# Dostenlinus/Aiyagari-HARK

Hardware: AMD Instinct MI355X
Metric: GE solves/sec (Table II sweep); agent-periods/sec; % HBM roofline (higher is better)
Workload: dtype f64

## Files before the change

### aiyagari_hark_amd/csrc/ge_resident.hip

```cpp
#include "common.h"
#include "egm_common.h"
#include "ge_search.h"
#include "hist_bicg.h"
#include "hist_cluster.h"
#include "internal.h"

#include <algorithm>
#include <cmath>

namespace aiy {

constexpr int kGeTHMax = 1024;
constexpr int kGeWavesMax = kGeTHMax / kWave;
constexpr int kGeMaxTiles = 16;
constexpr int kGeBufs = 5;
constexpr int kGeAaM = 3;
constexpr int kGeAaHist = kGeAaM + 2;
#ifdef AIY_DIAG_NO_FUSEA
constexpr bool kGeFuseA = false;
#else
constexpr bool kGeFuseA = true;
#endif
#ifndef AIY_FUSEA_KC2
#define AIY_FUSEA_KC2 0
#endif
constexpr bool kGeFuseAKc2 = AIY_FUSEA_KC2 != 0;
template <int NW>
constexpr size_t ge_egm_lds() { return (size_t)NW * (8 * kTile + 4 * kWin) * sizeof(double); }

struct GeCalDev {
  double alpha, delta, disc, r_lo, r_hi;
};

struct GeState;
struct GeRun {
  int n_cal, S, n_a, G, nj, cap, n_work;
  const double* a_grid;
  const double* P;
  const double* lab;
  const double* beta;
  const double* crra;
  const GeCalDev* cal;
  int method;
  double r_tol, egm_tol, hist_tol;
  int max_steps, max_cyc, max_hist;
  int warm_hist, warm_egm, secant, loose, extrap;
  int extrap_period;
  int aa_period;
  double* aah;
  int logsec;
  double loose_hist;
  double* qb;
  int* ainv;
  double* tab;
  double* mass;
  double* pmass;
  double* pg;
  int* lo;
  double* wlo;
  double* slab;
  int* span;
  unsigned* ctr;
  unsigned long long* gran;
  const int* cal_ids;
  GeState* saved;
  const int* resume;
  unsigned* done_ctr;
  int stop_at;
  int* out_done;
  unsigned* err;
  double* out_r;
  double* out_K;
  double* out_Ks;
  int* out_steps;
  int* out_cyc;
  int* out_its;
  int* out_status;
  double* out_prof;
  double* out_evlog;
};
constexpr int kGeProf = 8;
constexpr int kGeEvLog = 32;
constexpr int kGeEvRec = 6;

struct GeState {
  GeEval ev;
  GeEvalOpts opt;
  double Ks, dist, lam_prev, fext;
  int status, n, stop, nan_stop, moved, extrap;
  int in_hist;
  int buf[kGeBufs];
  long long cyc_sum, its_sum;
  unsigned long long t_egm, t_lot, t_hist, t_k, t0, t_ev0;
  unsigned nc_prev[2];
  unsigned nbc;
};

template <int TH>
__device__ __forceinline__ bool ge_reduce(unsigned long long* gran, int G, int w, unsigned& ne, const double* vals,
                                          int nv, unsigned kmax, double (*s_part)[kGeWavesMax], double* s_res,
                                          int* s_flag, unsigned* err) {
  asm volatile("s_waitcnt vmcnt(0)" ::: "memory");
  return hc_reduce<TH>(gran, G, w, ne, vals, nv, kmax, s_part, s_res, s_flag, err, [] {});
}

template <int SMAX, int NW, typename Sink, typename Begin, typename End>
__device__ __forceinline__ void ge_rows_pass(int S, int n_a, int j0, int j1, const double* __restrict__ a_grid,
                                             const double* __restrict__ src_m, const double* __restrict__ src_c,
                                             double R, const double* s_Wl, int* s_hint, double* lds_win,
                                             Sink&& sink, Begin&& begin, End&& end) {
  const int tid = threadIdx.x, lane = tid & (kWave - 1);
  const int wv = __builtin_amdgcn_readfirstlane(tid / kWave);
  const int n = n_a, n1 = n_a + 1;
  const int ntile = (j1 - j0 + kTile - 1) / kTile;
  double* X = lds_win + (size_t)wv * 4 * kWin;
  double* Y = X + kWin;
  double* XB = X + 2 * kWin;
  double* YB = X + 3 * kWin;
#pragma unroll 1
  for (int tile = wv; tile < ntile; tile += NW) {
    const int jr = j0 + tile * kTile + lane;
    const int j = jr < j1 ? jr : j1 - 1;
    const double a = a_grid[j];
    int* hint = s_hint + tile * SMAX;
    auto fetch = [&](int r, RowWin& wn) {
      const int rr = r < S ? r : S - 1;
      load_win<true>(src_m + (size_t)rr * n1, src_c + (size_t)rr * n1, n, win_base(hint[rr], n1), lane, wn);
    };
    unsigned redo = 0u;
    auto step_unit = [&](int u, const RowWin& wa, const RowWin& wb) {
      const int ra = 2 * u, rb = 2 * u + 1;
      if (ra >= S) return;
      const bool has_b = rb < S;
      const int rbb = has_b ? rb : ra;
      const bool na = __any(stage_win(wa, n, X, Y, lane));
      const bool nb = __any(stage_win(wb, n, XB, YB, lane));
      __builtin_amdgcn_fence(__ATOMIC_RELEASE, "wavefront");
      __builtin_amdgcn_wave_barrier();
      __builtin_amdgcn_fence(__ATOMIC_ACQUIRE, "wavefront");
      const double qa = R * a + s_Wl[ra];
      const double qb = R * a + s_Wl[rbb];
      int lba, lbb;
      bool oka, okb;
      const double fa = search_win(wa.base, na, n, qa, X, Y, lba, oka);
      const double fb = search_win(wb.base, nb, n, qb, XB, YB, lbb, okb);
      hint[ra] = __builtin_amdgcn_readfirstlane(lba);
      if (has_b) hint[rb] = __builtin_amdgcn_readfirstlane(lbb);
      if (__any(!oka)) redo |= 1u << ra;
      else sink(tile, jr, j, ra, qa, fa);
      if (has_b) {
        if (__any(!okb)) redo |= 1u << rb;
        else sink(tile, jr, j, rb, qb, fb);
      }
    };
    RowWin a0, b0, a1, b1;
    fetch(0, a0);
    fetch(1, b0);
    begin(tile, j);
#pragma unroll 1
    for (int u = 0; 2 * u < S; u += 2) {
      fetch(2 * u + 2, a1);
      fetch(2 * u + 3, b1);
      step_unit(u, a0, b0);
      fetch(2 * u + 4, a0);
      fetch(2 * u + 5, b0);
      step_unit(u + 1, a1, b1);
    }
#pragma unroll 1
    while (redo != 0u) {
      const int s = __builtin_ctz(redo);
      redo &= redo - 1u;
      const double q = R * a + s_Wl[s];
      int lb;
      const double f = interp_row_global_agent(src_m + (size_t)s * n1, src_c + (size_t)s * n1, n, q, lb);
      hint[s] = __builtin_amdgcn_readfirstlane(lb);
      sink(tile, jr, j, s, q, f);
    }
    end(tile, j, a);
  }
// ... 450 lines not shown
  pf[1] = st.t_lot * 0.01;
  pf[2] = st.t_hist * 0.01;
  pf[3] = st.t_k * 0.01;
  pf[4] = (__builtin_amdgcn_s_memrealtime() - st.t0) * 0.01;
  pf[5] = (double)st.cyc_sum;
  pf[6] = (double)st.its_sum;
  pf[7] = (double)st.ev.steps;
}

template <int SMAX, int SC, int KC, int TH, bool PULL>
__global__ __launch_bounds__(TH) void ge_cluster_kernel(GeRun g) {
  constexpr int NW = TH / kWave;
  static_assert(SMAX <= kGeSmax, "file-scope LDS sized for kGeSmax states");
  GeState& st = ge_st;

  const int per = gridDim.x >> 3;
  const int u = (blockIdx.x & 7) * per + (blockIdx.x >> 3);
  if (u >= g.n_work) return;
  const int G = g.G, S = g.S, n_a = g.n_a;
  const int tid = threadIdx.x;
  GeCtx cx;
  cx.G = G; cx.S = S; cx.n_a = n_a;
  cx.lc = u / G; cx.w = u - cx.lc * G;
  const int lc = cx.lc, w = cx.w, cal = g.cal_ids[lc];
  cx.cal = cal;
  cx.j0 = w * g.nj; cx.j1 = min(cx.j0 + g.nj, n_a);
  const int j0 = cx.j0, j1 = cx.j1;
  cx.a_grid = g.a_grid + (size_t)cal * n_a;
  cx.beta = g.beta[cal]; cx.gam = g.crra[cal];
  const GeCalDev cd = g.cal[cal];
  cx.tab_sz = (size_t)S * (n_a + 1);
  cx.tab = g.tab + (size_t)cal * kGeBufs * 2 * cx.tab_sz;
  const size_t row0 = (size_t)cal * S * n_a;
  cx.X = g.mass + row0;
  cx.PX = g.pmass + row0;
  cx.LO = g.lo + row0;
  cx.WL = g.wlo + row0;
  cx.ctr = g.ctr + (size_t)lc * kHcCtrStride;
  cx.cw = reinterpret_cast<unsigned long long*>(cx.ctr + 2);
  cx.gran = g.gran + (size_t)lc * 2 * G * kHcRedRec;
  cx.aah = g.aah + (size_t)cal * kGeAaHist * S * n_a;
  cx.err = g.err;
  unsigned nb = 0, ne = 0;
  const int pk = cx.gam == 1.0 ? 1 : (cx.gam == 3.0 ? 3 : (cx.gam == 5.0 ? 5 : 0));

  for (int q = tid; q < S * S; q += TH) ge_s_Pe[q] = g.P[(size_t)cal * S * S + q];
  for (int q = tid; q < kGeMaxTiles * SMAX; q += TH) ge_s_hint[q] = -1;
  if (tid == 0) {
    if (g.resume[cal]) {
      st = g.saved[cal];
      st.t0 = __builtin_amdgcn_s_memrealtime() - st.t0;
    } else {
      st.ev.init(ge_eval_opts(g), cd.r_lo, cd.r_hi);
      st.Ks = 0.0;
      st.in_hist = 0;
      st.status = 0;
      st.cyc_sum = st.its_sum = 0;
      for (int b = 0; b < kGeBufs; ++b) st.buf[b] = b;
      st.t_egm = st.t_lot = st.t_hist = st.t_k = 0ull;
      st.t0 = __builtin_amdgcn_s_memrealtime();
    }
    st.opt = ge_eval_opts(g);
    st.nc_prev[0] = st.nc_prev[1] = 0u;
    st.nbc = 0u;
  }
  __syncthreads();

  bool stopped = false;
  while ((!st.ev.rs.done && st.ev.steps < g.max_steps) || st.ev.final_ks) {
    if (g.stop_at > 0 && st.ev.steps > 0 && !st.in_hist) {
      unsigned flag = 0u, dlt = 0u;
      if (tid == 0)
        flag = __hip_atomic_load(to_global(g.done_ctr), __ATOMIC_RELAXED, __HIP_MEMORY_SCOPE_AGENT) >=
                       (unsigned)g.stop_at ? 1u : 0u;
      if (!ge_vote(cx, g.err, flag, dlt)) return;
      if (tid == 0) st.stop = dlt != 0u;
      __syncthreads();
      if (st.stop) {
        stopped = true;
        break;
      }
    }
    unsigned long long tp = __builtin_amdgcn_s_memrealtime();
    if (tid == 0 && !st.in_hist) st.t_ev0 = tp;
    if (!st.in_hist) {
      if (tid == 0) {
        st.ev.plan(st.opt, cd.alpha, cd.delta);
        st.extrap = g.extrap;
        st.moved = 0;
      }
      __syncthreads();
      if (tid < S) ge_s_Wl[tid] = st.ev.wage * g.lab[(size_t)cal * S + tid];
      const double R = st.ev.R, theta = st.ev.theta;
      const bool secant = st.ev.secant != 0, warm = st.ev.warm_egm != 0;
      const int b_cur = st.buf[2], b_prev = st.buf[3], b_init = st.buf[4];
      if (secant) ge_secant_tables<TH>(cx, b_cur, b_prev, b_init, theta);
      tp = __builtin_amdgcn_s_memrealtime();
      GeHhArgs ha;
      ha.tab = to_global(cx.tab); ha.aah = to_global(cx.aah); ha.ctr = to_global(cx.ctr); ha.err = to_global(g.err);
      ha.gran = to_global(cx.gran); ha.a_grid = to_global(cx.a_grid);
      ha.init_m = to_global((const double*)(secant ? cx.tabm(b_init) : (warm ? cx.tabm(b_cur) : nullptr)));
      ha.init_c = to_global((const double*)(secant ? cx.tabc(b_init) : (warm ? cx.tabc(b_cur) : nullptr)));
      ha.beta = cx.beta; ha.gam = cx.gam; ha.R = R;
      ha.j0 = j0; ha.j1 = j1; ha.w = w; ha.G = G; ha.S = S; ha.n_a = n_a;
      ha.opt = {g.max_cyc, g.aa_period, g.extrap_period};
      ha.dyn_lds = hk_lds_addr(ge_dyn);
      const int final_buf = pk == 1   ? ge_household_isolated<SMAX, SC, 1, TH>(ha, &nb, &ne)
                            : pk == 3 ? ge_household_isolated<SMAX, SC, 3, TH>(ha, &nb, &ne)
                            : pk == 5 ? ge_household_isolated<SMAX, SC, 5, TH>(ha, &nb, &ne)
                                      : ge_household_isolated<SMAX, SC, 0, TH>(ha, &nb, &ne);
      if (final_buf < 0) return;
      if (tid == 0) {
        const unsigned long long tn = __builtin_amdgcn_s_memrealtime();
        st.t_egm += tn - tp;
        st.cyc_sum += st.n;
        const int fb = final_buf;
        const int other = st.buf[0] == fb ? st.buf[1] : st.buf[0];
        const int old_prev = st.buf[3];
        st.buf[3] = st.buf[2];
        st.buf[2] = fb;
        st.buf[0] = other;
        st.buf[1] = old_prev;
      }
      __syncthreads();
      tp = __builtin_amdgcn_s_memrealtime();
      ge_lottery_fn<SMAX, NW>(S, n_a, j0, j1, cx.a_grid, cx.tabm(st.buf[2]), cx.tabc(st.buf[2]), R, st.ev.steps > 0,
                              cx.LO, cx.WL, PULL);
      ge_mass_start<TH>(cx, st.ev.fresh_mass != 0, warm, secant, theta);
      __syncthreads();
      if (tid == 0) {
        const unsigned long long tn = __builtin_amdgcn_s_memrealtime();
        st.t_lot += tn - tp;
        tp = tn;
      }
    }
    int mv;
    {
      HkArgs hk;
      hk.G = G; hk.S = S; hk.n_a = n_a; hk.cap = g.cap; hk.w = w; hk.j0 = j0; hk.j1 = j1;
      hk.LO = to_global((const int*)cx.LO); hk.WL = to_global((const double*)cx.WL); hk.X = to_global(cx.X);
      hk.Pg = to_global(g.pg + row0); hk.Vg = to_global((double*)nullptr);
      hk.slab_cl = to_global(g.slab + (size_t)lc * G * 2 * g.cap);
      hk.span_cl = to_global(g.span + (size_t)lc * G * SMAX * 4);
      hk.ctr = to_global(cx.ctr); hk.gran = to_global(cx.gran); hk.Pc = to_global(g.P + (size_t)cal * S * S);
      hk.max_iter = g.max_hist; hk.err = to_global(g.err);
      hk.tol = st.ev.htol;
      hk.stop_ctr = to_global((const unsigned*)(g.stop_at > 0 ? g.done_ctr : nullptr));
      hk.stop_at = (unsigned)g.stop_at;
      hk.Qg = to_global(g.qb + row0);
      hk.Ainv = to_global(g.ainv + (size_t)cal * S * (n_a + 1));
      hk.lottery_fresh = true;
      hk.dyn_lds = hk_lds_addr(ge_dyn);
      if constexpr (PULL) mv = hk_solve_inlined<SMAX, KC, TH, true, false, SC>(hk, &nb, &ne);
      else mv = hk_solve_isolated<SMAX, KC, TH, false, (KC == 1 || kGeFuseAKc2) && kGeFuseA, SC>(hk, &nb, &ne);
    }
    if (mv == -1) return;
    if (tid == 0) {
      const unsigned long long tn = __builtin_amdgcn_s_memrealtime();
      st.t_hist += tn - tp;
      tp = tn;
    }
    if (mv <= -2) {
      if (tid == 0) {
        st.its_sum += -mv - 2;
        st.in_hist = 1;
        if (w == 0) __hip_atomic_fetch_add(to_global(g.done_ctr + 1), 1u, __ATOMIC_RELAXED, __HIP_MEMORY_SCOPE_AGENT);
      }
      __syncthreads();
      stopped = true;
      break;
    }
    if (tid == 0) st.in_hist = 0;
    if (!ge_capital<TH>(cx, ne, g.err)) return;
    const bool fin = st.ev.final_ks != 0;
    if (tid == 0) {
      const double Ks = ge_s_res[0];
      if (w == 0 && st.ev.steps < kGeEvLog && !fin) {
        double* ev = g.out_evlog + ((size_t)cal * kGeEvLog + st.ev.steps) * kGeEvRec;
        ev[0] = st.ev.rs.x;
        ev[1] = (Ks - st.ev.Kd) / st.ev.Kd;
        ev[2] = (double)st.n;
        ev[3] = (double)mv;
        ev[4] = (double)st.ev.loose;
        ev[5] = (double)(__builtin_amdgcn_s_memrealtime() - st.t_ev0) * 0.01;
      }
      st.its_sum += mv;
      if (mv >= g.max_hist) st.status |= 2;
    }
    if (fin) {
      if (tid == 0) st.Ks = ge_s_res[0];
      __syncthreads();
      break;
    }
    if (tid == 0) {
      st.ev.accept(ge_s_res[0]);
      st.Ks = ge_s_res[0];
      st.t_k += __builtin_amdgcn_s_memrealtime() - tp;
    }
    __syncthreads();
  }
  if (stopped) {
    if (w == 0 && tid == 0) {
      st.t0 = __builtin_amdgcn_s_memrealtime() - st.t0;
      g.saved[cal] = st;
      g.out_done[cal] = 0;
    }
    return;
  }
  if (w == 0 && tid == 0) ge_write_out(cx, g, cd);
}

struct GePlan {
  int G = 0, nj = 0, kc = 0, smax = 0, sc = 0, cap = 0, blocks = 0, th = 0;
  size_t lds = 0;
  const void* fn = nullptr;
};

template <int SMAX, int SC, int KC, int TH>
static const void* ge_fn(bool pull) {
  return pull ? reinterpret_cast<const void*>(ge_cluster_kernel<SMAX, SC, KC, TH, true>)
              : reinterpret_cast<const void*>(ge_cluster_kernel<SMAX, SC, KC, TH, false>);
}

static bool ge_make_plan(aiy_handle* h, int n_cal, int S, int n_a, GePlan& p) {
  if (S < 1 || S > kGeSmax || n_a < 2 || n_cal < 1) return false;
  int cus = 0;
  if (hipDeviceGetAttribute(&cus, hipDeviceAttributeMultiprocessorCount, h->device) != hipSuccess || cus < 1) return false;
  if (h->cu_limit > 0) cus = std::min(cus, h->cu_limit);
  const int g_min = (n_a + 2 * 512 - 1) / (2 * 512);
  if (g_min > kHcMaxG || g_min > cus) return false;
  const int g_cap = h->hist_cluster_cap > 0 ? h->hist_cluster_cap : 32;
  int G = std::max(g_min, std::min(std::min(g_cap, kHcMaxG), cus / n_cal));
  G = std::min(G, n_a);
  p.nj = (n_a + G - 1) / G;
  p.G = (n_a + p.nj - 1) / p.nj;
  if (p.G > kHcMaxG) return false;
  if (p.nj > kGeMaxTiles * kTile) return false;
  if ((long long)p.G * n_cal > cus) return false;
  p.th = 512;
  const int th = p.th;
  p.kc = p.nj <= th ? 1 : 2;
  p.smax = S == 7 ? 7 : 8;
  p.sc = S == 7 ? 7 : 0;
  const bool pull = h->hist_pull != 0;
  if (p.sc == 7) p.fn = p.kc == 1 ? ge_fn<7, 7, 1, 512>(pull) : ge_fn<7, 7, 2, 512>(pull);
  else p.fn = p.kc == 1 ? ge_fn<8, 0, 1, 512>(pull) : ge_fn<8, 0, 2, 512>(pull);
  hipFuncAttributes fa;
  if (hipFuncGetAttributes(&fa, p.fn) != hipSuccess) return false;
  int lds_dev = 0;
  if (hipDeviceGetAttribute(&lds_dev, hipDeviceAttributeMaxSharedMemoryPerMultiprocessor, h->device) != hipSuccess)
    return false;
  const size_t lds_total = std::min<size_t>(kHcLdsTotal, (size_t)lds_dev);
  const size_t stat = fa.sharedSizeBytes;
  if (stat + 4096 >= lds_total) return false;
  p.lds = (lds_total - stat - 1024) / 256 * 256;
  const size_t vbytes = (size_t)p.kc * p.smax * th * sizeof(double);
  const size_t egm_lds = ge_egm_lds<8>();
  if (p.lds < egm_lds || p.lds <= vbytes + 4096) return false;
  p.cap = (int)((p.lds - vbytes) / sizeof(double));
  p.blocks = (p.G * n_cal + 7) / 8 * 8;
  return true;
}

struct GeScratch {
  size_t tab, mass, pmass, pg, qb, ainv, lo, wlo, slab, span, ctr, gran, ids, saved, resume, done, err, cal, outd, outi, prof,
      evlog, aah, bytes;
};
static GeScratch ge_scratch_layout(int n_cal, int S, int n_a, int cus, int cap_max) {
  GeScratch L;
  size_t o = 0;
  auto take = [&](size_t bytes) { const size_t at = o; o += (bytes + 255) / 256 * 256; return at; };
  const size_t pts = (size_t)n_cal * S * n_a;
  L.tab = take((size_t)n_cal * kGeBufs * 2 * S * (n_a + 1) * sizeof(double));
  L.mass = take(pts * 8); L.pmass = take(pts * 8); L.pg = take(pts * 8); L.qb = take(pts * 8);
  L.ainv = take((size_t)n_cal * S * (n_a + 1) * sizeof(int));
  L.lo = take(pts * 4); L.wlo = take(pts * 8);
  L.slab = take((size_t)cus * 2 * cap_max * sizeof(double));
  L.span = take((size_t)cus * 8 * 4 * sizeof(int));
  L.ctr = take((size_t)n_cal * kHcCtrStride * sizeof(unsigned));
  L.gran = take((size_t)cus * 2 * kHcRedRec * sizeof(unsigned long long));
  L.ids = take((size_t)n_cal * sizeof(int));
  L.saved = take((size_t)n_cal * sizeof(GeState));
  L.resume = take((size_t)n_cal * sizeof(int));
  L.done = take((size_t)n_cal * sizeof(int));
  L.err = take(256);
  L.cal = take((size_t)n_cal * sizeof(GeCalDev));
  L.outd = take((size_t)n_cal * 3 * sizeof(double));
  L.outi = take((size_t)n_cal * 4 * sizeof(int));
  L.prof = take((size_t)n_cal * kGeProf * sizeof(double));
  L.evlog = take((size_t)n_cal * kGeEvLog * kGeEvRec * sizeof(double));
  L.aah = take((size_t)n_cal * kGeAaHist * S * n_a * sizeof(double));
  L.bytes = o;
  return L;
}

int32_t ge_stationary_resident(aiy_handle* h, const aiy_stationary_model* M, const aiy_ge_options* o, double* r_out,
                               double* K_out, double* Ks_out, int32_t* steps_out, int32_t* cyc_out,
                               int32_t* its_out, int32_t* status_out, hipStream_t st) {
  if (!h->ge_resident || o->accel >= 0) return 0;
  const int n_cal = M->n_cal, S = M->S, n_a = M->n_a;
  GePlan p0;
  if (!ge_make_plan(h, n_cal, S, n_a, p0)) return 0;
  int cus = 0;
  if (hipDeviceGetAttribute(&cus, hipDeviceAttributeMultiprocessorCount, h->device) != hipSuccess) return 0;
  if (h->cu_limit > 0) cus = std::min(cus, h->cu_limit);
  const int cap_max = (int)(kHcLdsTotal / sizeof(double));
  const GeScratch L = ge_scratch_layout(n_cal, S, n_a, cus, cap_max);
// ... 208 lines not shown
```

### aiyagari_hark_amd/csrc/hist_bicg.h

```cpp
#pragma once

#include "common.h"
#include "hist_cluster.h"

namespace aiy {

constexpr int kHkStall = 256;
constexpr double kHkStopSentinel = 1e300;
constexpr int kHkHeavy = 31;
#ifndef AIY_HK_WAVE_CN
#define AIY_HK_WAVE_CN 6
#endif
constexpr int kHkWaveCn = AIY_HK_WAVE_CN;
static_assert(kHcCand <= 32, "covering-span index and count packed in 5 + 6 bits");
__device__ __forceinline__ unsigned short hk_cinfo(int cf, int cn, int hi) {
  return (unsigned short)(cf | (cn << 5) | (hi << 11));
}
__device__ __forceinline__ int hk_cf(int ci) { return ci & 31; }
__device__ __forceinline__ int hk_cn(int ci) { return (ci >> 5) & 63; }
__device__ __forceinline__ int hk_hi(int ci) { return ci >> 11; }

__device__ __forceinline__ double hk_uni(double x) {
  const unsigned long long u = (unsigned long long)__double_as_longlong(x);
  const unsigned lo = (unsigned)__builtin_amdgcn_readfirstlane((int)(unsigned)u);
// ... 544 lines not shown
            const int n1c = a2[u] - a1[u], n0c = a1[u] - a0[u];
            const bool heavy = valid && (n1c + n0c) > kWave;
            double acc = 0.0;
            if (valid && !heavy) {
              if (n1c > 0) acc += wv[u][0] * qv[u][0];
              if (n1c > 1) acc += wv[u][1] * qv[u][1];
              for (int j = a1[u] + 2; j < a2[u]; ++j) acc += w_at(sr, j) * q_at(sr, j);
              if (n0c > 0) acc += (1.0 - wv[u][2]) * qv[u][2];
              if (n0c > 1) acc += (1.0 - wv[u][3]) * qv[u][3];
              for (int j = a0[u] + 2; j < a1[u]; ++j) acc += (1.0 - w_at(sr, j)) * q_at(sr, j);
            }
            unsigned long long hm = __ballot(heavy);
            while (hm) {
              const int h = __builtin_ctzll(hm);
              hm &= hm - 1ull;
              const int b0 = __builtin_amdgcn_readlane(a0[u], h), b1 = __builtin_amdgcn_readlane(a1[u], h),
                        b2 = __builtin_amdgcn_readlane(a2[u], h);
              double pa = 0.0, pb = 0.0;
              for (int j = b1 + lane; j < b2; j += kWave) pa += w_at(sr, j) * q_at(sr, j);
              for (int j = b0 + lane; j < b1; j += kWave) pb += (1.0 - w_at(sr, j)) * q_at(sr, j);
              const double ta = wave_sum_lane63(pa), tb = wave_sum_lane63(pb);
              const double tot = __shfl(ta, kWave - 1, kWave) + __shfl(tb, kWave - 1, kWave);
              if (lane == h) acc = tot;
            }
            T[sr] = acc;
          }
        }
      }
#pragma unroll
      for (int sp = 0; sp < SMAX; ++sp) {
        double pc[SMAX];
        asm volatile("" ::: "memory");
#pragma unroll
        for (int s = 0; s < SMAX; ++s) pc[s] = s_P[s * SMAX + sp];
        double acc = 0.0;
#pragma unroll
        for (int s = 0; s < SMAX; ++s) acc += pc[s] * T[s];
        out[k][sp] = acc;
      }
    }
  };
  auto matvec = [&](const double (&q)[KC][SMAX], double (&out)[KC][SMAX]) -> bool {
    if constexpr (PULL) {
      HK_PH(5);
      stage_q(q);
      HK_PH(1);
      if (!barrier()) return false;
      HK_PH(2);
      pull_mix(out);
      HK_PH(3);
      return true;
    }
    HK_PH(5);
    push(q);
    HK_PH(0);
    const int par = (int)((nb + 1) & 1);
    publish(par);
    HK_PH(1);
    if (!barrier()) return false;
    HK_PH(2);
    gather_mix(par, out);
    HK_PH(3);
    return true;
  };
  auto reduce = [&](double (&vals)[kHcRed], int nv, unsigned kmax, auto&& prefetch) -> bool {
    HK_PH(5);
    hc_wave_parts(vals, nv, kmax, s_part);
    __syncthreads();
    ++ne;
    const unsigned long long tag = hc_red_tag(ne);
    unsigned long long* slot = hc_red_slot(gran, G, ne);
    hc_store_granules<TH>(slot, w, tag, nv, kmax, s_part);
    prefetch();
    if (wid == 0) hc_sweep(slot, G, tag, nv, kmax, s_res, &s_flag, err);
    __syncthreads();
    HK_PH(4);
    return s_flag != 0;
  };
  auto matvec_rp = [&](auto&& do_push, double (&out)[KC][SMAX], const double* vals, int nv, unsigned kmax) -> bool {
    HK_PH(5);
    hc_wave_parts(vals, nv, kmax, s_part);
    do_push();
    HK_PH(0);
    ++ne;
    const unsigned long long tag = hc_red_tag(ne);
    unsigned long long* slot = hc_red_slot(gran, G, ne);
    hc_store_granules<TH>(slot, w, tag, nv, kmax, s_part);
    const int par = (int)((nb + 1) & 1);
    publish(par);
    HK_PH(1);
    if (!barrier()) return false;
    HK_PH(2);
    if (wid == TH / kWave - 1) hc_sweep(slot, G, tag, nv, kmax, s_res, L.s_rok, err);
    gather_mix(par, out);
    __syncthreads();
    HK_PH(3);
    return *L.s_rok != 0;
  };
  auto matvec_r = [&](const double (&q)[KC][SMAX], double (&out)[KC][SMAX], const double* vals, int nv,
                      unsigned kmax) -> bool { return matvec_rp([&] { push(q); }, out, vals, nv, kmax); };
  double rv[KC][SMAX], pv[KC][SMAX], tv[KC][SMAX];
  double* Vl = kVlds ? Tacc + cap : (double*)r.Vg;
  double* Pg = (double*)r.Pg;
  auto vidx = [&](int k, int s) { return (k * SMAX + s) * TH + tid; };
  double part[kHcRed];
  const double tol = r.tol;
  int mv = 0;
  bool restart = true, first = true;
  double rho = 0.0, total0 = 0.0;
  auto own = [&](int jc, int k, int s) { return s < S && jc + k * TH < j1; };
  auto col_act = [&](int jc, bool (&act)[KC]) {
#pragma unroll
    for (int k = 0; k < KC; ++k) act[k] = jc + k * TH < j1;
  };
  bool act[KC];
  unsigned seed = 0;
  auto rh_at = [&](int jc, int k, int s) { return hk_rhat((unsigned)(s * n_a + jc + k * TH) + seed * 0x5BD1E995u); };
  double best = __builtin_inf();
  int mv_best = 0;
  auto gidx = [&](int jc, int k, int s) { return (size_t)s * n_a + jc + k * TH; };
  double* Ug = (double*)r.Qg;
  double pu = 0.0;
  auto make_u = [&]() {
    if constexpr (FUSEA) {
      const int jc = col();
      double acc = 0.0;
#pragma unroll
      for (int k = 0; k < KC; ++k)
#pragma unroll
        for (int s = 0; s < SMAX; ++s) {
          if (own(jc, k, s)) {
            int d;
            double wl;
            if constexpr (kLoReg) {
              d = dreg[k][s];
              wl = wreg[k][s];
            } else {
              d = LO[gidx(jc, k, s)];
              wl = WL[gidx(jc, k, s)];
            }
            double tr = 0.0;
            for (int sp = 0; sp < S; ++sp) {
              const unsigned q = (unsigned)(sp * n_a + d) + seed * 0x5BD1E995u;
              tr += s_P[s * SMAX + sp] * (wl * hk_rhat(q) + (1.0 - wl) * hk_rhat(q + 1u));
            }
            const double u = rh_at(jc, k, s) - tr;
            Ug[gidx(jc, k, s)] = u;
            acc += u * pv[k][s];
          }
        }
      pu = acc;
    }
  };
#ifndef AIY_FUSEA_KC2
#define AIY_FUSEA_KC2 0
#endif
  constexpr bool kUqPre = KC == 1 || AIY_FUSEA_KC2 == 1;
  HK_PH(-1);
  while (true) {
    if (restart) {
      int jc = col();
#pragma unroll
      for (int k = 0; k < KC; ++k)
#pragma unroll
        for (int s = 0; s < SMAX; ++s) {
          const double xv = X[min(s, S - 1) * n_a + min(jc + k * TH, n_a - 1)];
          pv[k][s] = own(jc, k, s) ? xv : 0.0;
        }
      if (!matvec(pv, tv)) return -1;
      ++mv;
      jc = col();
      double rr = 0.0, rm = 0.0, xs = 0.0;
#pragma unroll
      for (int k = 0; k < KC; ++k)
#pragma unroll
        for (int s = 0; s < SMAX; ++s) {
          rv[k][s] = tv[k][s] - pv[k][s];
          if (own(jc, k, s)) {
            rr += rh_at(jc, k, s) * rv[k][s];
            rm = nan_max(rm, fabs(rv[k][s]));
            xs += pv[k][s];
          }
        }
      part[0] = rr;
      part[1] = rm;
      part[2] = xs;
      if (!reduce(part, 3, 2u, [] {})) return -1;
      rho = s_res[0];
      if (mv == 1) total0 = s_res[2];
      if (s_res[1] < tol || mv >= r.max_iter) {
        const double scale = total0 / s_res[2];
#pragma unroll
        for (int k = 0; k < KC; ++k)
#pragma unroll
          for (int s = 0; s < SMAX; ++s)
            if (own(jc, k, s)) X[gidx(jc, k, s)] = mv == 1 ? tv[k][s] : tv[k][s] * scale;
        break;
      }
#pragma unroll
      for (int k = 0; k < KC; ++k)
#pragma unroll
        for (int s = 0; s < SMAX; ++s) pv[k][s] = rv[k][s];
      make_u();
      restart = false;
      first = true;
    }
#pragma unroll
    for (int k = 0; k < KC; ++k)
#pragma unroll
      for (int s = 0; s < SMAX; ++s) Vl[vidx(k, s)] = rv[k][s];
    if (r.stop_ctr != nullptr && tid == 0 && ((mv >> 1) & 7) == 0)
      s_stop = __hip_atomic_load((const unsigned*)r.stop_ctr, __ATOMIC_RELAXED, __HIP_MEMORY_SCOPE_AGENT) >= r.stop_at;
    double xq[KC][SMAX];
    int jc;
    if constexpr (FUSEA) {
      jc = col();
      col_act(jc, act);
      double rm = 0.0;
#pragma unroll
      for (int k = 0; k < KC; ++k) {
        if (act[k]) {
#pragma unroll
          for (int s = 0; s < SMAX; ++s)
            if (s < S) rm = nan_max(rm, fabs(Vl[vidx(k, s)]));
        }
        if constexpr (KC == 1) {
#pragma unroll
          for (int s = 0; s < SMAX; ++s) xq[k][s] = X[min(s, S - 1) * n_a + min(jc + k * TH, n_a - 1)];
        }
      }
      part[0] = pu;
      part[1] = (r.stop_ctr != nullptr && tid == 0 && s_stop) ? kHkStopSentinel : rm;
      if (!matvec_r(pv, tv, part, 2, 2u)) return -1;
      ++mv;
      jc = col();
#pragma unroll
      for (int k = 0; k < KC; ++k)
#pragma unroll
        for (int s = 0; s < SMAX; ++s) {
          const double v = pv[k][s] - tv[k][s];
          rv[k][s] = Vl[vidx(k, s)];
          Vl[vidx(k, s)] = v;
          if constexpr (KC > 1) xq[k][s] = X[min(s, S - 1) * n_a + min(jc + k * TH, n_a - 1)];
        }
    } else {
      if (!matvec(pv, tv)) return -1;
      ++mv;
      jc = col();
      col_act(jc, act);
      double rvv = 0.0, rm = 0.0;
#pragma unroll
      for (int k = 0; k < KC; ++k) {
#pragma unroll
        for (int s = 0; s < SMAX; ++s) {
          tv[k][s] = pv[k][s] - tv[k][s];
          rv[k][s] = Vl[vidx(k, s)];
          Vl[vidx(k, s)] = tv[k][s];
        }
        if (act[k]) {
#pragma unroll
          for (int s = 0; s < SMAX; ++s)
            if (s < S) {
              rvv += rh_at(jc, k, s) * tv[k][s];
              rm = nan_max(rm, fabs(rv[k][s]));
            }
        }
      }
      part[0] = rvv;
      part[1] = (r.stop_ctr != nullptr && tid == 0 && s_stop) ? kHkStopSentinel : rm;
      if (!reduce(part, 2, 2u, [&] {
            const int jq = col();
#pragma unroll
            for (int k = 0; k < KC; ++k)
#pragma unroll
              for (int s = 0; s < SMAX; ++s) xq[k][s] = X[min(s, S - 1) * n_a + min(jq + k * TH, n_a - 1)];
          }))
        return -1;
    }
    if (s_res[1] >= kHkStopSentinel) return -(2 + mv);
    if ((!first && s_res[1] < tol) || mv >= r.max_iter) {
      restart = true;
      continue;
    }
    if (first || s_res[1] < 0.9 * best) {
      best = first ? __builtin_inf() : s_res[1];
      mv_best = mv;
    } else if (mv - mv_best > kHkStall) {
      ++seed;
      best = __builtin_inf();
      restart = true;
      continue;
    }
    first = false;
    const double alpha = rho / s_res[0];
    if (!(fabs(alpha) < 1e300)) {
      restart = true;
      continue;
    }
    jc = col();
    col_act(jc, act);
#pragma unroll
    for (int k = 0; k < KC; ++k) {
      if (act[k]) {
#pragma unroll
        for (int s = 0; s < SMAX; ++s)
          if (s < S) {
            const int g = s * n_a + jc + k * TH;
            X[g] = xq[k][s] + alpha * pv[k][s];
            Pg[g] = pv[k][s];
          }
      }
#pragma unroll
      for (int s = 0; s < SMAX; ++s) rv[k][s] -= alpha * Vl[vidx(k, s)];
    }
    if (!matvec(rv, tv)) return -1;
    ++mv;
    jc = col();
    col_act(jc, act);
    double ts = 0.0, tt = 0.0, rs = 0.0, rt = 0.0, sm = 0.0;
#pragma unroll
    for (int k = 0; k < KC; ++k) {
#pragma unroll
      for (int s = 0; s < SMAX; ++s) tv[k][s] = rv[k][s] - tv[k][s];
      if (act[k]) {
#pragma unroll
        for (int s = 0; s < SMAX; ++s)
          if (s < S) {
            const double h = rh_at(jc, k, s);
            ts += tv[k][s] * rv[k][s];
            tt += tv[k][s] * tv[k][s];
            rs += h * rv[k][s];
            rt += h * tv[k][s];
            sm = nan_max(sm, fabs(rv[k][s]));
          }
      }
    }
    part[0] = ts;
    part[1] = tt;
    part[2] = rs;
    part[3] = rt;
    part[4] = sm;
    double pq[KC][SMAX];
    double uq[FUSEA && kUqPre ? KC : 1][SMAX];
    if (!reduce(part, 5, 16u, [&] {
          const int jq = col();
#pragma unroll
          for (int k = 0; k < KC; ++k)
#pragma unroll
            for (int s = 0; s < SMAX; ++s) {
              const int g = min(s, S - 1) * n_a + min(jq + k * TH, n_a - 1);
              xq[k][s] = X[g];
              pq[k][s] = Pg[g];
              if constexpr (FUSEA && kUqPre) uq[k][s] = Ug[g];
            }
        }))
      return -1;
    double omega = (s_res[4] < tol) ? 0.0 : s_res[0] / s_res[1];
    if (!(fabs(omega) < 1e300)) omega = 0.0;
    if (omega == 0.0) {
      restart = true;
      continue;
    }
    const double rho2 = s_res[2] - omega * s_res[3];
    const double beta = (rho2 / rho) * (alpha / omega);
    rho = rho2;
    jc = col();
    col_act(jc, act);
    double pun = 0.0;
#pragma unroll
    for (int k = 0; k < KC; ++k) {
      if (act[k]) {
#pragma unroll
        for (int s = 0; s < SMAX; ++s)
          if (s < S) X[s * n_a + jc + k * TH] = xq[k][s] + omega * rv[k][s];
      }
#pragma unroll
      for (int s = 0; s < SMAX; ++s) {
        const double pold = (act[k] && s < S) ? pq[k][s] : 0.0;
        rv[k][s] = rv[k][s] - omega * tv[k][s];
        pv[k][s] = rv[k][s] + beta * (pold - omega * Vl[vidx(k, s)]);
      }
      if constexpr (FUSEA && kUqPre) {
        if (act[k]) {
#pragma unroll
          for (int s = 0; s < SMAX; ++s)
            if (s < S) pun += uq[k][s] * pv[k][s];
        }
      }
    }
    if constexpr (FUSEA && !kUqPre) {
      double ul[KC][SMAX];
#pragma unroll
      for (int k = 0; k < KC; ++k)
#pragma unroll
        for (int s = 0; s < SMAX; ++s) ul[k][s] = Ug[min(s, S - 1) * n_a + min(jc + k * TH, n_a - 1)];
#pragma unroll
      for (int k = 0; k < KC; ++k)
#pragma unroll
        for (int s = 0; s < SMAX; ++s)
          if (own(jc, k, s)) pun += ul[k][s] * pv[k][s];
    }
    pu = pun;
    if (!(fabs(beta) < 1e300) || rho == 0.0) restart = true;
  }
#ifdef AIY_DIAG_PHASES
  if (tid == 0 && blockIdx.x >= AIY_DIAG_PHASES && blockIdx.x < AIY_DIAG_PHASES + 10 && mv > 0)
    printf("[bicg phases] block %d G=%d nj=%d matvecs=%d us/matvec: push %.2f publish %.2f barrier %.2f gather+mix "
           "%.2f reduce %.2f vector %.2f\n",
           (int)blockIdx.x, G, j1 - j0, mv, ph[0] * 0.01 / mv, ph[1] * 0.01 / mv, ph[2] * 0.01 / mv, ph[3] * 0.01 / mv,
           ph[4] * 0.01 / mv, ph[5] * 0.01 / mv);
#endif
  return mv;
}

__device__ __forceinline__ int hk_uni(int x) { return __builtin_amdgcn_readfirstlane(x); }
template <class T>
__device__ __forceinline__ gptr<T> hk_uni(gptr<T> p) {
  const unsigned long long u = (unsigned long long)p;
  const unsigned lo = (unsigned)__builtin_amdgcn_readfirstlane((int)(unsigned)u);
  const unsigned hi = (unsigned)__builtin_amdgcn_readfirstlane((int)(unsigned)(u >> 32));
  return (gptr<T>)(((unsigned long long)hi << 32) | lo);
}
__device__ __forceinline__ HkArgs hk_uniform_args(const HkArgs& a) {
  HkArgs u;
  u.G = hk_uni(a.G); u.S = hk_uni(a.S); u.n_a = hk_uni(a.n_a); u.cap = hk_uni(a.cap);
  u.w = hk_uni(a.w); u.j0 = hk_uni(a.j0); u.j1 = hk_uni(a.j1);
  u.LO = hk_uni(a.LO); u.WL = hk_uni(a.WL); u.X = hk_uni(a.X); u.Pg = hk_uni(a.Pg); u.Vg = hk_uni(a.Vg);
  u.slab_cl = hk_uni(a.slab_cl); u.span_cl = hk_uni(a.span_cl); u.ctr = hk_uni(a.ctr); u.gran = hk_uni(a.gran);
  u.Pc = hk_uni(a.Pc);
  u.tol = hk_uni(a.tol);
  u.max_iter = hk_uni(a.max_iter);
  u.err = hk_uni(a.err);
  u.stop_ctr = hk_uni(a.stop_ctr);
  u.stop_at = (unsigned)hk_uni((int)a.stop_at);
  u.Qg = hk_uni(a.Qg); u.Ainv = hk_uni(a.Ainv);
  u.lottery_fresh = hk_uni((int)a.lottery_fresh) != 0;
  u.dyn_lds = (unsigned)hk_uni((int)a.dyn_lds);
  return u;
}

template <int SMAX, int KC, int TH, bool PULL = false, bool FUSEA = false, int SC = 0>
__device__ __noinline__ int hk_solve_isolated(HkArgs a, unsigned* nb_io, unsigned* ne_io);
template <int SMAX, int KC, int TH, bool PULL = false, bool FUSEA = false, int SC = 0>
__device__ __forceinline__ int hk_solve_inlined(HkArgs a, unsigned* nb_io, unsigned* ne_io) {
  extern __shared__ double hk_dyn_in[];
  __shared__ int s_base[SMAX];
  __shared__ int s_pub[2 * SMAX][2];
  __shared__ int s_tot;
  __shared__ HcCand s_cand[SMAX][kHcCand];
  __shared__ int s_ncand[SMAX];
  __shared__ unsigned short s_cinfo[PULL ? 1 : KC * SMAX * TH];
  __shared__ double s_P[SMAX * SMAX];
  __shared__ double s_part[kHcRed][TH / kWave];
  __shared__ double s_res[kHcRed];
  __shared__ int s_flag, s_stop;
  __shared__ int s_ex[2 * SMAX];
  __shared__ int s_nheavy, s_heavy[kHkHeavy][4], s_rok, s_wcnt[TH / kWave];
  __shared__ double s_hval[kHkHeavy];
  HkShared<SMAX, KC, TH> L{hk_dyn_in, s_base, s_pub, &s_tot, s_cand, s_ncand, s_cinfo, s_P, s_part, s_res,
                                 &s_flag, &s_stop, s_ex, &s_nheavy, s_wcnt, s_heavy, s_hval, &s_rok};
  unsigned nb = *nb_io, ne = *ne_io;
  const int mv = hk_solve<SMAX, KC, TH, PULL, FUSEA, SC>(a, L, nb, ne);
  *nb_io = nb;
  *ne_io = ne;
  return mv;
}
template <int SMAX, int KC, int TH, bool PULL, bool FUSEA, int SC>
__device__ __noinline__ int hk_solve_isolated(HkArgs a, unsigned* nb_io, unsigned* ne_io) {
  double* hk_dyn = (double*)(lptr<double>)(size_t)(unsigned)__builtin_amdgcn_readfirstlane((int)a.dyn_lds);
  __shared__ int s_base[SMAX];
  __shared__ int s_pub[2 * SMAX][2];
  __shared__ int s_tot;
  __shared__ HcCand s_cand[SMAX][kHcCand];
  __shared__ int s_ncand[SMAX];
  __shared__ unsigned short s_cinfo[KC * SMAX * TH];
  __shared__ double s_P[SMAX * SMAX];
  __shared__ double s_part[kHcRed][TH / kWave];
  __shared__ double s_res[kHcRed];
  __shared__ int s_flag, s_stop;
  __shared__ int s_ex[2 * SMAX];
  __shared__ int s_nheavy, s_heavy[kHkHeavy][4], s_rok, s_wcnt[TH / kWave];
  __shared__ double s_hval[kHkHeavy];
  HkShared<SMAX, KC, TH> L{hk_dyn, s_base, s_pub, &s_tot, s_cand, s_ncand, s_cinfo, s_P, s_part, s_res,
                                 &s_flag, &s_stop, s_ex, &s_nheavy, s_wcnt, s_heavy, s_hval, &s_rok};
  unsigned nb = *nb_io, ne = *ne_io;
  const int mv = hk_solve<SMAX, KC, TH, PULL, FUSEA, SC>(hk_uniform_args(a), L, nb, ne);
  *nb_io = nb;
  *ne_io = ne;
  return mv;
}

}
```

Before: 618.5.

## Enable fused BiCGSTAB for KC>1 using atomic adds to X instead of register copies

For KC>1 the fused variant is now always enabled. X updates go through relaxed agent-scope atomic fetch-adds rather than preloading X into registers and writing xq+alpha*p. This removes the per-iteration X loads and their register array, and the U vector prefetch inside the reduction is now used for all KC. The cost is global atomics on X and an explicit vmcnt wait plus agent-coherent loads on restart, which could add memory latency or contention.

After: 614.4. About the same (-0.7%).

```diff
diff --git a/aiyagari_hark_amd/csrc/ge_resident.hip b/aiyagari_hark_amd/csrc/ge_resident.hip
--- a/aiyagari_hark_amd/csrc/ge_resident.hip
+++ b/aiyagari_hark_amd/csrc/ge_resident.hip
@@ -21,10 +21,6 @@
 #else
 constexpr bool kGeFuseA = true;
 #endif
-#ifndef AIY_FUSEA_KC2
-#define AIY_FUSEA_KC2 0
-#endif
-constexpr bool kGeFuseAKc2 = AIY_FUSEA_KC2 != 0;
 template <int NW>
 constexpr size_t ge_egm_lds() { return (size_t)NW * (8 * kTile + 4 * kWin) * sizeof(double); }
 
@@ -781,7 +777,7 @@
       hk.lottery_fresh = true;
       hk.dyn_lds = hk_lds_addr(ge_dyn);
       if constexpr (PULL) mv = hk_solve_inlined<SMAX, KC, TH, true, false, SC>(hk, &nb, &ne);
-      else mv = hk_solve_isolated<SMAX, KC, TH, false, (KC == 1 || kGeFuseAKc2) && kGeFuseA, SC>(hk, &nb, &ne);
+      else mv = hk_solve_isolated<SMAX, KC, TH, false, kGeFuseA, SC>(hk, &nb, &ne);
     }
     if (mv == -1) return;
     if (tid == 0) {
diff --git a/aiyagari_hark_amd/csrc/hist_bicg.h b/aiyagari_hark_amd/csrc/hist_bicg.h
--- a/aiyagari_hark_amd/csrc/hist_bicg.h
+++ b/aiyagari_hark_amd/csrc/hist_bicg.h
@@ -720,19 +720,18 @@
       pu = acc;
     }
   };
-#ifndef AIY_FUSEA_KC2
-#define AIY_FUSEA_KC2 0
-#endif
-  constexpr bool kUqPre = KC == 1 || AIY_FUSEA_KC2 == 1;
+  constexpr bool kXAdd = FUSEA && KC > 1;
   HK_PH(-1);
   while (true) {
     if (restart) {
       int jc = col();
+      if constexpr (kXAdd) asm volatile("s_waitcnt vmcnt(0)" ::: "memory");
 #pragma unroll
       for (int k = 0; k < KC; ++k)
 #pragma unroll
         for (int s = 0; s < SMAX; ++s) {
-          const double xv = X[min(s, S - 1) * n_a + min(jc + k * TH, n_a - 1)];
+          const double* xp = &X[min(s, S - 1) * n_a + min(jc + k * TH, n_a - 1)];
+          const double xv = (kXAdd && mv > 0) ? load_f64_agent(xp) : *xp;
           pv[k][s] = own(jc, k, s) ? xv : 0.0;
         }
       if (!matvec(pv, tv)) return -1;
@@ -779,7 +778,7 @@
       for (int s = 0; s < SMAX; ++s) Vl[vidx(k, s)] = rv[k][s];
     if (r.stop_ctr != nullptr && tid == 0 && ((mv >> 1) & 7) == 0)
       s_stop = __hip_atomic_load((const unsigned*)r.stop_ctr, __ATOMIC_RELAXED, __HIP_MEMORY_SCOPE_AGENT) >= r.stop_at;
-    double xq[KC][SMAX];
+    double xq[kXAdd ? 1 : KC][SMAX];
     int jc;
     if constexpr (FUSEA) {
       jc = col();
@@ -809,7 +808,6 @@
           const double v = pv[k][s] - tv[k][s];
           rv[k][s] = Vl[vidx(k, s)];
           Vl[vidx(k, s)] = v;
-          if constexpr (KC > 1) xq[k][s] = X[min(s, S - 1) * n_a + min(jc + k * TH, n_a - 1)];
         }
     } else {
       if (!matvec(pv, tv)) return -1;
@@ -874,7 +872,9 @@
         for (int s = 0; s < SMAX; ++s)
           if (s < S) {
             const int g = s * n_a + jc + k * TH;
-            X[g] = xq[k][s] + alpha * pv[k][s];
+            if constexpr (kXAdd)
+              __hip_atomic_fetch_add(to_global(&X[g]), alpha * pv[k][s], __ATOMIC_RELAXED, __HIP_MEMORY_SCOPE_AGENT);
+            else X[g] = xq[k][s] + alpha * pv[k][s];
             Pg[g] = pv[k][s];
           }
       }
@@ -909,7 +909,7 @@
     part[3] = rt;
     part[4] = sm;
     double pq[KC][SMAX];
-    double uq[FUSEA && kUqPre ? KC : 1][SMAX];
+    double uq[FUSEA ? KC : 1][SMAX];
     if (!reduce(part, 5, 16u, [&] {
           const int jq = col();
 #pragma unroll
@@ -917,9 +917,9 @@
 #pragma unroll
             for (int s = 0; s < SMAX; ++s) {
               const int g = min(s, S - 1) * n_a + min(jq + k * TH, n_a - 1);
-              xq[k][s] = X[g];
+              if constexpr (!kXAdd) xq[k][s] = X[g];
               pq[k][s] = Pg[g];
-              if constexpr (FUSEA && kUqPre) uq[k][s] = Ug[g];
+              if constexpr (FUSEA) uq[k][s] = Ug[g];
             }
         }))
       return -1;
@@ -940,7 +940,12 @@
       if (act[k]) {
 #pragma unroll
         for (int s = 0; s < SMAX; ++s)
-          if (s < S) X[s * n_a + jc + k * TH] = xq[k][s] + omega * rv[k][s];
+          if (s < S) {
+            const int g = s * n_a + jc + k * TH;
+            if constexpr (kXAdd)
+              __hip_atomic_fetch_add(to_global(&X[g]), omega * rv[k][s], __ATOMIC_RELAXED, __HIP_MEMORY_SCOPE_AGENT);
+            else X[g] = xq[k][s] + omega * rv[k][s];
+          }
       }
 #pragma unroll
       for (int s = 0; s < SMAX; ++s) {
@@ -948,25 +953,13 @@
         rv[k][s] = rv[k][s] - omega * tv[k][s];
         pv[k][s] = rv[k][s] + beta * (pold - omega * Vl[vidx(k, s)]);
       }
-      if constexpr (FUSEA && kUqPre) {
+      if constexpr (FUSEA) {
         if (act[k]) {
 #pragma unroll
           for (int s = 0; s < SMAX; ++s)
             if (s < S) pun += uq[k][s] * pv[k][s];
         }
       }
-    }
-    if constexpr (FUSEA && !kUqPre) {
-      double ul[KC][SMAX];
-#pragma unroll
-      for (int k = 0; k < KC; ++k)
-#pragma unroll
-        for (int s = 0; s < SMAX; ++s) ul[k][s] = Ug[min(s, S - 1) * n_a + min(jc + k * TH, n_a - 1)];
-#pragma unroll
-      for (int k = 0; k < KC; ++k)
-#pragma unroll
-        for (int s = 0; s < SMAX; ++s)
-          if (own(jc, k, s)) pun += ul[k][s] * pv[k][s];
     }
     pu = pun;
     if (!(fabs(beta) < 1e300) || rho == 0.0) restart = true;
```
